# OpenSim2Real/gym-os2r

Hardware: AMD Instinct MI355X
Metric: env-steps/sec (aggregate) monopod balance task (higher is better)
Workload: dtype f64; 1 GPU; C4: 65536 envs/GPU free_hip balancing, ground contact, per-env domain randomisation (C5 = 8 x C4); envs_per_gpu=65536, total_envs=65536, task_mode=free_hip, substeps=10, pgs_exact=12, preroll_steps=1000, contact=True, domain_randomisation=True, actions=U(-1,1) Philox on device, n_ranks_seen=1, splits=1, rollout_steps_per_launch=1

## Files before the change

### gym-os2r_amd/csrc/os2r_device.hpp

```cpp
#pragma once
#include <type_traits>
#include <hip/hip_runtime.h>
#include <stdint.h>

#include "../../include/os2r.h"
#include "os2r_models_gen.hpp"

namespace os2r {

constexpr int kWave = 64;
template <typename T> struct StdSolver { static constexpr int kNormalIters = 2; static constexpr bool kExact = true; };
template <> struct StdSolver<float> { static constexpr int kNormalIters = 2; static constexpr bool kExact = false; };
__host__ __device__ constexpr int warm_first(int) { return 3; }
__host__ __device__ constexpr int sweep_cap_base(int nq) { return nq >= 5 ? 6 : 4; }
constexpr int kExactRounds = 8;
constexpr unsigned kCarryJoints = 0x80000000u;
template <typename T, int NQ_> struct SolverCarry {
  unsigned act = 0u;
  T ln[NQ_] = {}, lx[NQ_] = {}, ly[NQ_] = {}, lf[NQ_] = {};
};
template <typename T> __host__ __device__ constexpr int std_iters(int nq) { return sizeof(T) == 8 ? sweep_cap_base(nq) + kExactRounds : 20; }
template <typename T> __host__ __device__ inline bool is_std_solver(int iters, int normal_iters, int exact, int nq) {
  return iters == std_iters<T>(nq) && normal_iters == StdSolver<T>::kNormalIters && (exact > 0) == StdSolver<T>::kExact;
}
// ... 240 lines not shown
template <typename T> __device__ __forceinline__ T comp(V3<T> a, int k) { return k == 0 ? a.x : (k == 1 ? a.y : a.z); }
template <typename T> __device__ __forceinline__ void add_comp(V3<T>& a, int k, T v) {
  if (k == 0) a.x += v; else if (k == 1) a.y += v; else a.z += v;
}
template <typename T> __device__ __forceinline__ V3<T> rmul(const T (&R)[9], V3<T> v) {
  return {R[0] * v.x + R[1] * v.y + R[2] * v.z, R[3] * v.x + R[4] * v.y + R[5] * v.z, R[6] * v.x + R[7] * v.y + R[8] * v.z};
}
template <typename T> __device__ __forceinline__ V3<T> rtmul(const T (&R)[9], V3<T> v) {
  return {R[0] * v.x + R[3] * v.y + R[6] * v.z, R[1] * v.x + R[4] * v.y + R[7] * v.z, R[2] * v.x + R[5] * v.y + R[8] * v.z};
}

__device__ __forceinline__ double sqrt_t(double x) { return sqrt(x); }
__device__ __forceinline__ float sqrt_t(float x) { return sqrtf(x); }
__device__ __forceinline__ bool sincos_in_range(double x) { return fabs(x) < 8.2e5; }
__device__ __forceinline__ bool sincos_in_range(float x) { return fabsf(x) < 200.0f; }
__device__ __forceinline__ void sincos_lib(double x, double& s, double& c) { sincos(x, &s, &c); }
__device__ __forceinline__ void sincos_lib(float x, float& s, float& c) { sincosf(x, &s, &c); }
__device__ __forceinline__ void sincos_fast(float x, float& s, float& c) {
  const float k = __builtin_rintf(x * 0.636619772f);
  float r = __builtin_fmaf(-k, 1.5703125f, x);
  r = __builtin_fmaf(-k, 4.837512969970703125e-4f, r);
  r = __builtin_fmaf(-k, 7.54978995489188e-8f, r);
  const float z = r * r;
  float ps = -1.9515295891e-4f;
  ps = __builtin_fmaf(ps, z, 8.3321608736e-3f);
  ps = __builtin_fmaf(ps, z, -1.6666654611e-1f);
  const float sr = __builtin_fmaf(r * z, ps, r);
  float pc = 2.443315711809948e-5f;
  pc = __builtin_fmaf(pc, z, -1.388731625493765e-3f);
  pc = __builtin_fmaf(pc, z, 4.166664568298827e-2f);
  const float cr = __builtin_fmaf(z * z, pc, __builtin_fmaf(-0.5f, z, 1.0f));
  const int n = (int)k;
  const float a = (n & 1) ? cr : sr, b = (n & 1) ? sr : cr;
  s = (n & 2) ? -a : a;
  c = ((n + 1) & 2) ? -b : b;
}
__device__ __forceinline__ void sincos_fast(double x, double& s, double& c) {
  const double k = __builtin_rint(x * 0x1.45f306dc9c883p-1);
  double r = __builtin_fma(-k, 0x1.921fb54442d18p+0, x);
  r = __builtin_fma(-k, 0x1.1a62633145c07p-54, r);
  const double z = r * r;
  double ps = 0x1.5d93a5acfd57cp-33;
  ps = __builtin_fma(ps, z, -0x1.ae5e68a2b9cebp-26);
  ps = __builtin_fma(ps, z, 0x1.71de357b1fe7dp-19);
  ps = __builtin_fma(ps, z, -0x1.a01a019c161d5p-13);
  ps = __builtin_fma(ps, z, 0x1.111111110f8a6p-7);
  ps = __builtin_fma(ps, z, -0x1.5555555555549p-3);
  const double sr = __builtin_fma(r * z, ps, r);
  double pc = -0x1.8fae9be8838d4p-37;
  pc = __builtin_fma(pc, z, 0x1.1ee9ebdb4b1c4p-29);
  pc = __builtin_fma(pc, z, -0x1.27e4f809c52adp-22);
  pc = __builtin_fma(pc, z, 0x1.a01a019cb1590p-16);
  pc = __builtin_fma(pc, z, -0x1.6c16c16c15177p-10);
  pc = __builtin_fma(pc, z, 0x1.555555555554cp-5);
  const double cr = __builtin_fma(z * z, pc, __builtin_fma(-0.5, z, 1.0));
  const int n = (int)k;
  const double a = (n & 1) ? cr : sr, b = (n & 1) ? sr : cr;
  s = (n & 2) ? -a : a;
  c = ((n + 1) & 2) ? -b : b;
}

__device__ __forceinline__ double rcp_t(double x) {
  double r = __builtin_amdgcn_rcp(x);
  r = __builtin_fma(__builtin_fma(-x, r, 1.0), r, r);
  r = __builtin_fma(__builtin_fma(-x, r, 1.0), r, r);
  return r;
}
__device__ __forceinline__ float rcp_t(float x) {
  float r = __builtin_amdgcn_rcpf(x);
  return __builtin_fmaf(__builtin_fmaf(-x, r, 1.0f), r, r);
}
__device__ __forceinline__ double rsqrt_t(double x) {
  double r = __builtin_amdgcn_rsq(x);
  r = r * __builtin_fma(-0.5 * x * r, r, 1.5);
  r = r * __builtin_fma(-0.5 * x * r, r, 1.5);
  return r;
}
__device__ __forceinline__ float rsqrt_t(float x) {
  float r = __builtin_amdgcn_rsqf(x);
  return r * __builtin_fmaf(-0.5f * x * r, r, 1.5f);
}

__device__ __forceinline__ double fmax_t(double a, double b) { return fmax(a, b); }
__device__ __forceinline__ float fmax_t(float a, float b) { return fmaxf(a, b); }
__device__ __forceinline__ double fmin_t(double a, double b) { return fmin(a, b); }
__device__ __forceinline__ float fmin_t(float a, float b) { return fminf(a, b); }
__device__ __forceinline__ double fma_t(double a, double b, double c) { return __builtin_fma(a, b, c); }
__device__ __forceinline__ float fma_t(float a, float b, float c) { return __builtin_fmaf(a, b, c); }
__device__ __forceinline__ double fabs_t(double x) { return fabs(x); }
__device__ __forceinline__ float fabs_t(float x) { return fabsf(x); }

__device__ __forceinline__ bool finite_t(double x) {
  asm volatile("" : "+v"(x));
  return ((__double_as_longlong(x) >> 52) & 0x7ff) != 0x7ff;
}
__device__ __forceinline__ bool finite_t(float x) {
  asm volatile("" : "+v"(x));
  return ((__float_as_int(x) >> 23) & 0xff) != 0xff;
}

template <typename T> __device__ __forceinline__ V3<T> symmul(const T (&S)[6], V3<T> v) {
  return {S[0] * v.x + S[1] * v.y + S[2] * v.z, S[1] * v.x + S[3] * v.y + S[4] * v.z, S[2] * v.x + S[4] * v.y + S[5] * v.z};
}

template <typename T>
struct ArtInertia {
  T A[6];
  T H[9];
  T M[6];
};

template <typename T> __device__ __forceinline__ void rot_general(const T (&R)[9], const T (&B)[9], T (&out)[9]) {
  T t[9];
#pragma unroll
  for (int i = 0; i < 3; ++i)
#pragma unroll
    for (int j = 0; j < 3; ++j) t[3 * i + j] = R[3 * i] * B[j] + R[3 * i + 1] * B[3 + j] + R[3 * i + 2] * B[6 + j];
#pragma unroll
  for (int i = 0; i < 3; ++i)
#pragma unroll
    for (int j = 0; j < 3; ++j) out[3 * i + j] = t[3 * i] * R[3 * j] + t[3 * i + 1] * R[3 * j + 1] + t[3 * i + 2] * R[3 * j + 2];
}
template <typename T> __device__ __forceinline__ void rot_sym(const T (&R)[9], const T (&S)[6], T (&out)[6]) {
  const T B[9] = {S[0], S[1], S[2], S[1], S[3], S[4], S[2], S[4], S[5]};
  T t[9];
#pragma unroll
  for (int i = 0; i < 3; ++i)
#pragma unroll
    for (int j = 0; j < 3; ++j) t[3 * i + j] = R[3 * i] * B[j] + R[3 * i + 1] * B[3 + j] + R[3 * i + 2] * B[6 + j];
  int k = 0;
#pragma unroll
  for (int i = 0; i < 3; ++i)
#pragma unroll
    for (int j = i; j < 3; ++j) out[k++] = t[3 * i] * R[3 * j] + t[3 * i + 1] * R[3 * j + 1] + t[3 * i + 2] * R[3 * j + 2];
}

template <typename T, typename MD, bool DR>
struct Params;
template <typename T, typename MD>
struct Params<T, MD, false> {
  MD m;
  T g;
  __device__ __forceinline__ T mass(int i) const { return m.mass(i); }
  __device__ __forceinline__ T damping(int i) const { return m.damping(i); }
  __device__ __forceinline__ T friction(int i) const { return m.friction(i); }
  __device__ __forceinline__ T mu(int i) const { return m.mu(i); }
  __device__ __forceinline__ T gravity() const { return g; }
};
template <typename T, typename MD>
struct Params<T, MD, true> {
  MD m;
  const T* slots;
  T g;
  static constexpr int NQ = MD::NQ;
  __device__ __forceinline__ T mass(int i) const { return slots[(0 * NQ + i) * kWave]; }
  __device__ __forceinline__ T damping(int i) const { return slots[(1 * NQ + i) * kWave]; }
  __device__ __forceinline__ T friction(int i) const { return slots[(2 * NQ + i) * kWave]; }
  __device__ __forceinline__ T mu(int i) const { return slots[(3 * NQ + i) * kWave]; }
  __device__ __forceinline__ T gravity() const { return g; }
};

constexpr int kStamps = 32;
#if defined(OS2R_STAMPS) && defined(OS2R_STAMPS_LIGHT)
#define OS2R_STAMP(idx) do { } while (0)
#elif defined(OS2R_STAMPS)
#define OS2R_STAMP(idx)                                                                        \
  do {                                                                                         \
    __builtin_amdgcn_sched_barrier(0);                                                         \
    unsigned long long t_;                                                                     \
    asm volatile("s_memtime %0\n\ts_waitcnt lgkmcnt(0)" : "=s"(t_)::"memory");                 \
    __builtin_amdgcn_sched_barrier(0);                                                         \
    stamps[idx] += t_ - stamp_prev;                                                            \
    stamp_prev = t_;                                                                           \
  } while (0)
#elif defined(OS2R_PHASE_MARKS)
#define OS2R_STAMP(idx) asm volatile("s_nop 15\n\ts_nop %0\n\ts_nop %1" :: "i"((idx) % 8), "i"((idx) / 8) : "memory")
#else
#define OS2R_STAMP(idx) do { } while (0)
#endif

#ifdef OS2R_ISA_MARKS
#define OS2R_ISA_MARK(n) asm volatile("s_nop " #n ::: "memory")
#else
#define OS2R_ISA_MARK(n) do { } while (0)
#endif

constexpr int kPinVmem = 0x1 | 0x2 | 0x4 | 0x8 | 0x80 | 0x100 | 0x200 | 0x400;

constexpr int kPinDs = 0x1 | 0x2 | 0x4 | 0x8 | 0x10 | 0x20 | 0x40 | 0x400;

__device__ __forceinline__ double opaque(double x) { asm volatile("" : "+v"(x)); return x; }
__device__ __forceinline__ float opaque(float x) { asm volatile("" : "+v"(x)); return x; }

template <typename T> __device__ __forceinline__ T pick3(int k, T a, T b, T c) { return k == 0 ? a : (k == 1 ? b : c); }

template <typename T, typename MD>
__device__ __forceinline__ void joint_rotation(const MD& md, int i, T s_, T c_, T (&R)[9]) {
  const T s = opaque(s_), c = opaque(c_);
  const int ax = md.axis(i);
  const int ca = ax == 0 ? 1 : (ax == 1 ? 2 : 0);
  const int cb = ax == 0 ? 2 : (ax == 1 ? 0 : 1);
#pragma unroll
  for (int r = 0; r < 3; ++r) {
    const T fa = md.rfix(i, 3 * r + ca), fb = md.rfix(i, 3 * r + cb);
    const T keep = md.rfix(i, 3 * r + ax), va = c * fa + s * fb, vb = c * fb - s * fa;
#pragma unroll
    for (int j = 0; j < 3; ++j) R[3 * r + j] = j == ax ? keep : (j == ca ? va : vb);
  }
}

template <unsigned CMASK, int NB>
__device__ __forceinline__ constexpr int next_cand_body(int b) {
  for (int k = b + 1; k < NB; ++k)
    if ((CMASK >> k) & 1u) return k;
  return NB;
}
template <int B, int NB, unsigned CMASK, typename F>
__device__ __forceinline__ bool for_body(int b, F&& f) {
  if constexpr (B < NB) {
    if constexpr (((CMASK >> B) & 1u) && __builtin_popcount(CMASK >> B) <= 3) {
      if (b == B) { f(std::integral_constant<int, B>{}); return true; }
    }
    return for_body<B + 1, NB, CMASK>(b, f);
  } else {
    return false;
  }
}

enum { kSolverBoth = 0, kSolverExact = 1, kSolverSweeps = 2 };
template <typename T, typename MD, bool CONTACT, bool DR, bool COUNT = false, int SOLVER = kSolverBoth>
__device__ __forceinline__ void substep(const MD& md, const Params<T, MD, DR>& par,
                                        T (&q)[MD::NQ], T (&qd)[MD::NQ], T (&sn)[MD::NQ], T (&cs)[MD::NQ], bool first_iteration,
                                        T tau_hip, T tau_knee, T dt, T erp,
                                        T max_erv, T margin, int pgs_iters, int pgs_normal_iters, int pgs_exact, T pgs_tol, T* __restrict__ lds,
                                        const T* __restrict__ cand_lds, ModelPtr<T> mconst, WorkCounts& wc, SolverCarry<T, MD::NQ>& carry
#ifdef OS2R_STAMPS
                                        , unsigned long long (&stamps)[kStamps], unsigned long long& stamp_prev
#endif
                                        ) {
  constexpr int NQ = MD::NQ;
  constexpr unsigned CMASK = CONTACT ? MD::CMASK : 0u;
  const T inv_dt = rcp_t(dt);
  const T m_first = par.mass(NQ - 1), damp_first = par.damping(NQ - 1);
  __builtin_amdgcn_sched_barrier(DR ? kPinDs : kPinVmem);
  {
    bool ok = true, small = !first_iteration;
#pragma unroll
    for (int i = 0; i < NQ; ++i) { ok = ok && sincos_in_range(q[i]); small = small && fabs_t(dt * qd[i]) < T(0.06); }
    if constexpr (COUNT) wc.full_sincos += __ballot(!small) != 0ull ? 1u : 0u;
    if (small) {
#pragma unroll
      for (int i = 0; i < NQ; ++i) {
        const T d = dt * qd[i], z = d * d;
        T p = fma_t(z, T(-1.0 / 39916800.0), T(1.0 / 362880.0));
        p = fma_t(z, p, T(-1.0 / 5040.0));
        p = fma_t(z, p, T(1.0 / 120.0));
        p = fma_t(z, p, T(-1.0 / 6.0));
        const T sd = fma_t(d * z, p, d);
        T r = fma_t(z, T(-1.0 / 3628800.0), T(1.0 / 40320.0));
        r = fma_t(z, r, T(-1.0 / 720.0));
        r = fma_t(z, r, T(1.0 / 24.0));
        r = fma_t(z, r, T(-0.5));
        const T cm = z * r;
        const T s0 = sn[i], c0 = cs[i];
        sn[i] = s0 + fma_t(c0, sd, s0 * cm);
        cs[i] = c0 + fma_t(-s0, sd, c0 * cm);
      }
    } else if (ok) {
#pragma unroll
      for (int i = 0; i < NQ; ++i) sincos_fast(q[i], sn[i], cs[i]);
    } else {
#pragma unroll
      for (int i = 0; i < NQ; ++i) sincos_lib(q[i], sn[i], cs[i]);
    }
  }

  OS2R_STAMP(0);
  const int lane_ = threadIdx.x;
  auto L = [&](int slot) -> T& { return lds[slot * kWave + lane_]; };
  constexpr int kUa = 0, kUl = 3 * NQ, kDi = 6 * NQ, kU = 7 * NQ;
  auto ldv = [&](int base, int i) { return mk(L(base + 3 * i), L(base + 3 * i + 1), L(base + 3 * i + 2)); };
  auto stv = [&](int base, int i, V3<T> x) { L(base + 3 * i) = x.x; L(base + 3 * i + 1) = x.y; L(base + 3 * i + 2) = x.z; };

  V3<T> wv[NQ], vv[NQ];
  {
    V3<T> w = mk<T>(0, 0, 0), v = mk<T>(0, 0, 0);
#pragma unroll
    for (int i = 0; i < NQ; ++i) {
      if (i > 0) {
        const V3<T> r = mk(md.rpos(i, 0), md.rpos(i, 1), md.rpos(i, 2));
        T Ri[9];
        joint_rotation<T>(md, i, sn[i], cs[i], Ri);
        const V3<T> wn = rtmul(Ri, w);
        v = rtmul(Ri, v + cross(w, r));
        w = wn;
      }
      add_comp(w, md.axis(i), qd[i]);
      wv[i] = w;
      vv[i] = v;
    }
  }

  OS2R_STAMP(12);
  {
    ArtInertia<T> acc;
    V3<T> pn, pf;
    T m_next = m_first, damp_next = damp_first;
#pragma unroll
    for (int i = NQ - 1; i >= 0; --i) {
      const int ax = md.axis(i);
      const V3<T> w = wv[i], v = vv[i];
      const T m = m_next;
      const T damp = damp_next;
      if (i > 0) {
        m_next = par.mass(i - 1);
        damp_next = par.damping(i - 1);
        __builtin_amdgcn_sched_barrier(DR ? kPinDs : kPinVmem);
      }
      const V3<T> cm = mk(md.com(i, 0), md.com(i, 1), md.com(i, 2));
      const V3<T> h = m * cm;
      ArtInertia<T> I;
      I.A[0] = md.icom(i, 0) + m * (cm.y * cm.y + cm.z * cm.z);
      I.A[1] = md.icom(i, 1) - m * cm.x * cm.y;
      I.A[2] = md.icom(i, 2) - m * cm.x * cm.z;
      I.A[3] = md.icom(i, 3) + m * (cm.x * cm.x + cm.z * cm.z);
      I.A[4] = md.icom(i, 4) - m * cm.y * cm.z;
      I.A[5] = md.icom(i, 5) + m * (cm.x * cm.x + cm.y * cm.y);
      I.H[0] = 0; I.H[1] = -h.z; I.H[2] = h.y;
      I.H[3] = h.z; I.H[4] = 0; I.H[5] = -h.x;
      I.H[6] = -h.y; I.H[7] = h.x; I.H[8] = 0;
      I.M[0] = m; I.M[1] = 0; I.M[2] = 0; I.M[3] = m; I.M[4] = 0; I.M[5] = m;
      const V3<T> nI = symmul(I.A, w) + cross(h, v);
      const V3<T> fI = m * v - cross(h, w);
      V3<T> pAn = cross(w, nI) + cross(v, fI);
      V3<T> pAf = cross(w, fI);
      if (i < NQ - 1) {
#pragma unroll
        for (int k = 0; k < 6; ++k) { I.A[k] += acc.A[k]; I.M[k] += acc.M[k]; }
#pragma unroll
        for (int k = 0; k < 9; ++k) I.H[k] += acc.H[k];
        pAn = pAn + pn;
        pAf = pAf + pf;
      }
      const V3<T> Ua = mk(pick3(ax, I.A[0], I.A[1], I.A[2]), pick3(ax, I.A[1], I.A[3], I.A[4]), pick3(ax, I.A[2], I.A[4], I.A[5]));
      const V3<T> Ul = mk(pick3(ax, I.H[0], I.H[3], I.H[6]), pick3(ax, I.H[1], I.H[4], I.H[7]), pick3(ax, I.H[2], I.H[5], I.H[8]));
      const T D = comp(Ua, ax) + dt * damp;
      const T Dinv = rcp_t(D);
      T tau = T(0);
      if (i == md.act_dof(0)) tau = tau_hip;
      if (i == md.act_dof(1)) tau = tau_knee;
      const T u = tau - damp * qd[i] - comp(pAn, ax);
      stv(kUa, i, Ua);
      stv(kUl, i, Ul);
      L(kDi + i) = Dinv;
      L(kU + i) = u;
      if (i > 0) {
        const V3<T> ka = Dinv * Ua, kl = Dinv * Ul;
        ArtInertia<T> Ia;
        Ia.A[0] = I.A[0] - ka.x * Ua.x; Ia.A[1] = I.A[1] - ka.x * Ua.y; Ia.A[2] = I.A[2] - ka.x * Ua.z;
        Ia.A[3] = I.A[3] - ka.y * Ua.y; Ia.A[4] = I.A[4] - ka.y * Ua.z; Ia.A[5] = I.A[5] - ka.z * Ua.z;
        Ia.H[0] = I.H[0] - ka.x * Ul.x; Ia.H[1] = I.H[1] - ka.x * Ul.y; Ia.H[2] = I.H[2] - ka.x * Ul.z;
        Ia.H[3] = I.H[3] - ka.y * Ul.x; Ia.H[4] = I.H[4] - ka.y * Ul.y; Ia.H[5] = I.H[5] - ka.y * Ul.z;
        Ia.H[6] = I.H[6] - ka.z * Ul.x; Ia.H[7] = I.H[7] - ka.z * Ul.y; Ia.H[8] = I.H[8] - ka.z * Ul.z;
        Ia.M[0] = I.M[0] - kl.x * Ul.x; Ia.M[1] = I.M[1] - kl.x * Ul.y; Ia.M[2] = I.M[2] - kl.x * Ul.z;
        Ia.M[3] = I.M[3] - kl.y * Ul.y; Ia.M[4] = I.M[4] - kl.y * Ul.z; Ia.M[5] = I.M[5] - kl.z * Ul.z;
        V3<T> sq = mk<T>(0, 0, 0);
        add_comp(sq, ax, qd[i]);
        const V3<T> ca = cross(w, sq), cl = cross(v, sq);
        const V3<T> Hc = mk(Ia.H[0] * cl.x + Ia.H[1] * cl.y + Ia.H[2] * cl.z, Ia.H[3] * cl.x + Ia.H[4] * cl.y + Ia.H[5] * cl.z,
                            Ia.H[6] * cl.x + Ia.H[7] * cl.y + Ia.H[8] * cl.z);
        const V3<T> Htc = mk(Ia.H[0] * ca.x + Ia.H[3] * ca.y + Ia.H[6] * ca.z, Ia.H[1] * ca.x + Ia.H[4] * ca.y + Ia.H[7] * ca.z,
                             Ia.H[2] * ca.x + Ia.H[5] * ca.y + Ia.H[8] * ca.z);
        const T ud = u * Dinv;
        const V3<T> pan = pAn + symmul(Ia.A, ca) + Hc + ud * Ua;
        const V3<T> paf = pAf + Htc + symmul(Ia.M, cl) + ud * Ul;
        const V3<T> r = mk(md.rpos(i, 0), md.rpos(i, 1), md.rpos(i, 2));
        T Ri[9];
        joint_rotation<T>(md, i, sn[i], cs[i], Ri);
        T Ar[6], Hr[9], Mr[6];
        rot_sym(Ri, Ia.A, Ar);
        rot_general(Ri, Ia.H, Hr);
        rot_sym(Ri, Ia.M, Mr);
        const T Mf[9] = {Mr[0], Mr[1], Mr[2], Mr[1], Mr[3], Mr[4], Mr[2], Mr[4], Mr[5]};
        T Hs[9];
#pragma unroll
        for (int j = 0; j < 3; ++j) {
          const V3<T> col = cross(r, mk(Mf[j], Mf[3 + j], Mf[6 + j]));
          Hs[j] = Hr[j] + col.x; Hs[3 + j] = Hr[3 + j] + col.y; Hs[6 + j] = Hr[6 + j] + col.z;
        }
        V3<T> x0[3], x1[3];
#pragma unroll
        for (int k = 0; k < 3; ++k) {
          x0[k] = cross(r, mk(Hr[3 * k], Hr[3 * k + 1], Hr[3 * k + 2]));
          x1[k] = cross(r, mk(Hs[3 * k], Hs[3 * k + 1], Hs[3 * k + 2]));
        }
        acc.A[0] = Ar[0] + x0[0].x + x1[0].x;
        acc.A[1] = Ar[1] + x0[1].x + x1[0].y;
        acc.A[2] = Ar[2] + x0[2].x + x1[0].z;
        acc.A[3] = Ar[3] + x0[1].y + x1[1].y;
        acc.A[4] = Ar[4] + x0[2].y + x1[1].z;
        acc.A[5] = Ar[5] + x0[2].z + x1[2].z;
#pragma unroll
        for (int k = 0; k < 9; ++k) acc.H[k] = Hs[k];
#pragma unroll
        for (int k = 0; k < 6; ++k) acc.M[k] = Mr[k];
        pf = rmul(Ri, paf);
        pn = rmul(Ri, pan) + cross(r, pf);
      }
      OS2R_STAMP(13 + (NQ - 1 - i));
    }
  }

  T vs[NQ];
  T hu[2], hd[2];
  V3<T> hua[2], hul[2];
  {
    V3<T> aa = mk<T>(0, 0, 0), al = mk<T>(0, 0, -par.gravity());
    auto request = [&](int i, int b) { hu[b] = L(kU + i); hua[b] = ldv(kUa, i); hul[b] = ldv(kUl, i); hd[b] = L(kDi + i); };
    auto arrived = [&](int b) {
      asm volatile("" : "+v"(hu[b]), "+v"(hd[b]), "+v"(hua[b].x), "+v"(hua[b].y), "+v"(hua[b].z), "+v"(hul[b].x), "+v"(hul[b].y), "+v"(hul[b].z));
      asm volatile("" ::: "memory");
    };
    request(0, 0);
#pragma unroll
    for (int i = 0; i < NQ; ++i) {
      const int b = i & 1;
      arrived(b);
      if (i + 1 < NQ) request(i + 1, b ^ 1);
      const int ax = md.axis(i);
      const V3<T> r = mk(md.rpos(i, 0), md.rpos(i, 1), md.rpos(i, 2));
      V3<T> sq = mk<T>(0, 0, 0);
      add_comp(sq, ax, qd[i]);
      T Ri[9];
      joint_rotation<T>(md, i, sn[i], cs[i], Ri);
      const V3<T> pa_ = rtmul(Ri, aa);
      const V3<T> pl_ = rtmul(Ri, al + cross(aa, r));
      aa = pa_ + cross(wv[i], sq);
      al = pl_ + cross(vv[i], sq);
      const T qdd = (hu[b] - dot(hua[b], aa) - dot(hul[b], al)) * hd[b];
      add_comp(aa, ax, qdd);
      vs[i] = qd[i] + dt * qdd;
    }
  }

  OS2R_STAMP(1);
  constexpr int NB = NQ;
  constexpr int kLc = 0;
  auto Lcs = [&](int i, int k) -> T& { return L(kLc + i * (i + 1) / 2 + k); };
  T Lc[NQ][NQ];
  T Ldi[NQ];
  {
    T uk[NQ][NQ];
    V3<T> pn_[NQ], pf_[NQ];
    V3<T> mUa[2], mUl[2];
    T mdi[2];
    auto request_m = [&](int i, int b) { mUa[b] = ldv(kUa, i); mUl[b] = ldv(kUl, i); mdi[b] = L(kDi + i); };
    auto arrived_m = [&](int b) {
      asm volatile("" : "+v"(mdi[b]), "+v"(mUa[b].x), "+v"(mUa[b].y), "+v"(mUa[b].z), "+v"(mUl[b].x), "+v"(mUl[b].y), "+v"(mUl[b].z));
      asm volatile("" ::: "memory");
    };
    constexpr bool kAhead = sizeof(T) == 8;
    if constexpr (kAhead) { mUa[(NQ - 1) & 1] = hua[(NQ - 1) & 1]; mUl[(NQ - 1) & 1] = hul[(NQ - 1) & 1]; mdi[(NQ - 1) & 1] = hd[(NQ - 1) & 1]; }
#pragma unroll
    for (int i = NQ - 1; i >= 0; --i) {
      if constexpr (kAhead) {
        if (i < NQ - 1) arrived_m(i & 1);
        if (i > 0) { request_m(i - 1, (i - 1) & 1); __builtin_amdgcn_sched_barrier(kPinDs); }
      } else {
        request_m(i, i & 1);
      }
      const V3<T> Ua = mUa[i & 1], Ul = mUl[i & 1];
      const T di = mdi[i & 1];
      uk[i][i] = T(1);
      if (i < NQ - 1) {
        const V3<T> r = mk(md.rpos(i + 1, 0), md.rpos(i + 1, 1), md.rpos(i + 1, 2));
        T Ri[9];
        joint_rotation<T>(md, i + 1, sn[i + 1], cs[i + 1], Ri);
#pragma unroll
        for (int k = i + 1; k < NQ; ++k) {
          const V3<T> f = rmul(Ri, pf_[k]);
          const V3<T> n = rmul(Ri, pn_[k]) + cross(r, f);
          uk[k][i] = -comp(n, md.axis(i));
          if (i > 0) {
            const T s_ = uk[k][i] * di;
            pn_[k] = n + s_ * Ua;
            pf_[k] = f + s_ * Ul;
          }
        }
      }
      if (i > 0) {
        pn_[i] = di * Ua;
        pf_[i] = di * Ul;
      }
      Ldi[i] = rsqrt_t(di);
      const T sdi = di * Ldi[i];
#pragma unroll
      for (int r = i; r < NQ; ++r) Lc[r][i] = r == i ? sdi : uk[r][i] * sdi;
    }
  }
  OS2R_STAMP(19);

  OS2R_STAMP(2);
  T fb[NQ];
  T mub[NB];
#pragma unroll
  for (int j = 0; j < NQ; ++j) fb[j] = par.friction(j);
#pragma unroll
  for (int b = 0; b < NB; ++b) mub[b] = ((CMASK >> b) & 1u) ? par.mu(b) : T(0);
  __builtin_amdgcn_sched_barrier(DR ? kPinDs : kPinVmem);
  T y[NQ];
  T idj[NQ];
#pragma unroll
  for (int j = 0; j < NQ; ++j) {
    T mjj = 0;
#pragma unroll
    for (int k = 0; k <= j; ++k) { mjj += Lc[j][k] * Lc[j][k]; Lcs(j, k) = Lc[j][k]; }
    idj[j] = mjj > T(0) ? rcp_t(mjj) : T(0);
  }
#pragma unroll
  for (int i = 0; i < NQ; ++i) {
    T acc_ = vs[i];
#pragma unroll
    for (int k = 0; k < i; ++k) acc_ -= Lc[i][k] * y[k];
    y[i] = opaque(acc_ * Ldi[i]);
  }
  constexpr bool kStdExact = sizeof(T) == 8 && SOLVER == kSolverExact && MD::kStatic;
  constexpr bool kParkY0 = sizeof(T) == 8 && !kStdExact && (SOLVER != kSolverSweeps || !MD::kStatic);
  constexpr int kY0Slot = NQ * (NQ + 1) / 2 + 3 * NQ + NQ;
  static_assert(kY0Slot + NQ <= 8 * NQ, "per-lane LDS slots");
  T y0[NQ];
#pragma unroll
  for (int i = 0; i < NQ; ++i) {
    if constexpr (kParkY0) L(kY0Slot + i) = y[i];
    else y0[i] = y[i];
  }

  OS2R_STAMP(3);
  T dn[NB], dx[NB], dy[NB], erv[NB];
  T Gr[NB][3][NQ];
  bool act[NB];
  bool wave_act[NB];
#pragma unroll
  for (int b = 0; b < NB; ++b) { act[b] = false; wave_act[b] = false; }
  if (CMASK != 0u) {
    T Rw[9], ow[3];
    V3<T> aw[NQ], jo[NQ];
#pragma unroll
    for (int b = 0; b < NB; ++b) {
      constexpr int CHS = 4;
      T bA[3 * CHS], bB[3 * CHS];
      auto request = [&](int kk, int kend, T (&d)[3 * CHS]) {
#pragma unroll
        for (int j = 0; j < 3 * CHS; ++j) d[j] = (kk + j / 3 < kend) ? mconst->cand_p[kk + j / 3][j % 3] : T(0);
      };
      if constexpr (MD::kStatic) {
        if ((CMASK >> b) & 1u) {
          request(md.cand_begin(b), md.cand_begin(b + 1), bA);
          asm volatile("" ::: "memory");
        }
      }
      const V3<T> r = mk(md.rpos(b, 0), md.rpos(b, 1), md.rpos(b, 2));
      T Rb[9];
      joint_rotation<T>(md, b, sn[b], cs[b], Rb);
      if (b == 0) {
#pragma unroll
        for (int k = 0; k < 9; ++k) Rw[k] = Rb[k];
        ow[0] = r.x; ow[1] = r.y; ow[2] = r.z;
      } else {
        const V3<T> t = rmul(Rw, r);
        ow[0] += t.x; ow[1] += t.y; ow[2] += t.z;
        T n[9];
#pragma unroll
        for (int i = 0; i < 3; ++i)
#pragma unroll
          for (int j = 0; j < 3; ++j) n[3 * i + j] = Rw[3 * i] * Rb[j] + Rw[3 * i + 1] * Rb[3 + j] + Rw[3 * i + 2] * Rb[6 + j];
#pragma unroll
        for (int k = 0; k < 9; ++k) Rw[k] = n[k];
      }
      const int ax = md.axis(b);
      aw[b] = mk(pick3(ax, Rw[0], Rw[1], Rw[2]), pick3(ax, Rw[3], Rw[4], Rw[5]), pick3(ax, Rw[6], Rw[7], Rw[8]));
      jo[b] = mk(ow[0], ow[1], ow[2]);
      if (!((CMASK >> b) & 1u)) continue;
      OS2R_STAMP(4);
      const int k0 = md.cand_begin(b), k1 = md.cand_begin(b + 1);
      T W = 0, sx = 0, sy = 0, sz = 0;
      const T zc = Rw[6] * md.cand_center(b, 0) + Rw[7] * md.cand_center(b, 1) + Rw[8] * md.cand_center(b, 2) + ow[2];
      const bool near = zc - md.cand_radius(b) < margin;
      if constexpr (MD::kStatic) {
#pragma unroll
        for (int j = 0; j < 3 * CHS; ++j) asm volatile("" : "+s"(bA[j]));
        asm volatile("" ::: "memory");
      }
      if constexpr (COUNT) wc.scanned += __ballot(near) != 0ull ? 1u : 0u;
      if (__ballot(near) != 0ull)
      {
        constexpr int CH = 4;
        auto fetch = [&](int k, T (&d)[3 * CH]) {
#pragma unroll
          for (int j = 0; j < 3 * CH; ++j) d[j] = cand_lds[3 * k + j];
        };
        auto consume = [&](const T (&d)[3 * CH]) {
#pragma unroll
          for (int c = 0; c < CH; ++c) {
            const T px = d[3 * c], py = d[3 * c + 1], pz = d[3 * c + 2];
            const T z = Rw[6] * px + Rw[7] * py + Rw[8] * pz + ow[2];
            const T wgt = fmax_t(margin - z, T(0));
            W += wgt; sx += wgt * px; sy += wgt * py; sz += wgt * pz;
          }
        };
        if constexpr (MD::kStatic) {
          const T mo = margin - ow[2];
          auto arrived = [&](T (&d)[3 * CH]) {
#pragma unroll
            for (int j = 0; j < 3 * CH; ++j) asm volatile("" : "+s"(d[j]));
            asm volatile("" ::: "memory");
          };
          const int ga = MD::cand_group_axis(b), a1 = (ga + 1) % 3, a2 = (ga + 2) % 3;
          T S[3] = {T(0), T(0), T(0)};
          T Wg = T(0), pg = T(0), base = mo;
          auto weigh = [&](const T (&d)[3 * CH], int kk) {
#pragma unroll
            for (int c = 0; c < CH; ++c) {
              if (kk + c < k1) {
                if (MD::cand_starts_run(b, kk + c, ga)) {
                  W += Wg; S[ga] = fma_t(pg, Wg, S[ga]);
                  Wg = T(0); pg = d[3 * c + ga];
                  base = fma_t(-Rw[6 + ga], pg, mo);
                }
                const T p1 = d[3 * c + a1], p2 = d[3 * c + a2];
                const T mz = fma_t(-Rw[6 + a1], p1, fma_t(-Rw[6 + a2], p2, base));
                const T wgt = fmax_t(mz, T(0));
                Wg += wgt; S[a1] = fma_t(wgt, p1, S[a1]); S[a2] = fma_t(wgt, p2, S[a2]);
              }
            }
          };
          static_assert(CH == CHS, "chunk size of the request issued ahead");
#pragma unroll
          for (int kk = k0; kk < k1; kk += 2 * CH) {
            arrived(bA);
            if (kk + CH < k1) request(kk + CH, k1, bB);
            weigh(bA, kk);
            if (kk + CH < k1) {
              arrived(bB);
              if (kk + 2 * CH < k1) request(kk + 2 * CH, k1, bA);
              weigh(bB, kk + CH);
            }
          }
          W += Wg; S[ga] = fma_t(pg, Wg, S[ga]);
          sx = S[0]; sy = S[1]; sz = S[2];
        } else {
        T bufA[3 * CH], bufB[3 * CH];
        int k = k0;
        const int kpair = k0 + ((k1 - k0) / (2 * CH)) * (2 * CH);
        if (k < kpair) {
          fetch(k, bufA);
#pragma unroll 1
          for (; k < kpair; k += 2 * CH) {
            fetch(k + CH, bufB);
            consume(bufA);
            if (k + 2 * CH < kpair) fetch(k + 2 * CH, bufA);
            consume(bufB);
          }
        }
#pragma unroll 1
        for (; k < k1; ++k) {
          const T px = cand_lds[3 * k], py = cand_lds[3 * k + 1], pz = cand_lds[3 * k + 2];
          const T z = Rw[6] * px + Rw[7] * py + Rw[8] * pz + ow[2];
          const T wgt = fmax_t(margin - z, T(0));
          W += wgt; sx += wgt * px; sy += wgt * py; sz += wgt * pz;
        }
        }
      }
      OS2R_STAMP(5);
      act[b] = W > T(0);
      wave_act[b] = __ballot(act[b]) != 0ull;
      if constexpr (COUNT) { wc.row_bodies += wave_act[b] ? 1u : 0u; wc.lane_contacts += (unsigned)__popcll(__ballot(act[b])); }
      if (wave_act[b]) {
        T lcb[NQ][NQ];
#pragma unroll
        for (int j = 0; j < NQ; ++j)
#pragma unroll
          for (int k = 0; k < NQ; ++k)
            if (j <= b && k <= j) lcb[j][k] = Lcs(j, k);
        __builtin_amdgcn_sched_barrier(kPinDs);
        const T iw = act[b] ? rcp_t(W) : T(0);
        const V3<T> pc = mk(sx * iw, sy * iw, sz * iw);
        const V3<T> pw = rmul(Rw, pc) + jo[b];
        const T gap = pw.z;
        const T e = erp * (-gap) * inv_dt;
        erv[b] = gap >= T(0) ? -gap * inv_dt : (e > max_erv ? max_erv : e);
        T Jn[NQ], Jx[NQ], Jy[NQ];
#pragma unroll
        for (int j = 0; j < NQ; ++j) {
          if (j <= b) {
            const V3<T> c = cross(aw[j], pw - jo[j]);
            Jx[j] = c.x; Jy[j] = c.y; Jn[j] = c.z;
          }
        }
        T sdn = 0, sdx = 0, sdy = 0;
#pragma unroll
        for (int k = 0; k < NQ; ++k) {
          if (k <= b) {
            T gn = 0, gx = 0, gy = 0;
#pragma unroll
            for (int j = k; j < NQ; ++j)
              if (j <= b) { const T l = lcb[j][k]; gn += Jn[j] * l; gx += Jx[j] * l; gy += Jy[j] * l; }
            Gr[b][0][k] = gn; Gr[b][1][k] = gx; Gr[b][2][k] = gy;
            sdn += gn * gn; sdx += gx * gx; sdy += gy * gy;
          }
        }
        dn[b] = (act[b] && sdn > T(0)) ? rcp_t(sdn) : T(0);
        dx[b] = (act[b] && sdx > T(0)) ? rcp_t(sdx) : T(0);
        dy[b] = (act[b] && sdy > T(0)) ? rcp_t(sdy) : T(0);
      }
    }
  }

  OS2R_STAMP(6);
  T ln[NB], lx[NB], ly[NB], lf[NQ];
#pragma unroll
  for (int b = 0; b < NB; ++b) { ln[b] = 0; lx[b] = 0; ly[b] = 0; }
#pragma unroll
  for (int j = 0; j < NQ; ++j) lf[j] = 0;
#pragma unroll
  for (int j = 0; j < NQ; ++j) {
    fb[j] = opaque(fb[j] * dt);
    idj[j] = fb[j] > T(0) ? idj[j] : T(0);
  }

  T moved = T(0);
  auto contact_row = [&](int b, int row, T target, T rd, T& l, T lo, T hi, bool upper, bool measure) {
    T g[NQ];
    T res = -target;
#pragma unroll
    for (int k = 0; k < NQ; ++k)
      if (k <= b) { g[k] = Gr[b][row][k]; res = fma_t(g[k], y[k], res); }
    T lam = fma_t(-res, rd, l);
    lam = lam < lo ? lo : lam;
    if (upper) lam = lam > hi ? hi : lam;
    const T dl = lam - l;
    l = lam;
    if (measure) moved = fma_t(fabs_t(res), fabs_t(dl), moved);
#pragma unroll
    for (int k = 0; k < NQ; ++k)
      if (k <= b) y[k] = fma_t(g[k], dl, y[k]);
  };
  auto joint_rows = [&](bool measure) {
#pragma unroll
    for (int j = 0; j < NQ; ++j) {
      T res = Lc[j][0] * y[0];
#pragma unroll
      for (int k = 1; k < NQ; ++k)
        if (k <= j) res = fma_t(Lc[j][k], y[k], res);
      T lam = fma_t(-res, idj[j], lf[j]);
// ... 436 lines not shown
```

Before: 494.7 million env-steps/s.

## Fuse mass-matrix factor computation into the articulated-inertia inward pass

For static f64 models with domain randomisation and four DOFs, the Cholesky-like factor (Lc, Ldi) is now built during the backward articulated-body sweep. Propagated unit-force columns are transformed alongside the inertia accumulation, so the separate second inward pass is skipped, along with its reloads of Ua/Ul/Dinv from the scratch store. The cost is higher register pressure from carrying the cuk, cpn and cpf arrays through the sweep, which could hurt occupancy.

```diff
diff --git a/gym-os2r_amd/csrc/os2r_device.hpp b/gym-os2r_amd/csrc/os2r_device.hpp
--- a/gym-os2r_amd/csrc/os2r_device.hpp
+++ b/gym-os2r_amd/csrc/os2r_device.hpp
@@ -566,6 +566,11 @@
   }
 
   OS2R_STAMP(12);
+  constexpr bool kFusedInward = sizeof(T) == 8 && MD::kStatic && DR && NQ == 4;
+  T Lc[NQ][NQ];
+  T Ldi[NQ];
+  T cuk[NQ][NQ];
+  V3<T> cpn[NQ], cpf[NQ];
   {
     ArtInertia<T> acc;
     V3<T> pn, pf;
@@ -618,6 +623,27 @@
       stv(kUl, i, Ul);
       L(kDi + i) = Dinv;
       L(kU + i) = u;
+      if constexpr (kFusedInward) {
+        cuk[i][i] = T(1);
+#pragma unroll
+        for (int k = i + 1; k < NQ; ++k) {
+          const V3<T> n = cpn[k], f = cpf[k];
+          cuk[k][i] = -comp(n, ax);
+          if (i > 0) {
+            const T s_ = cuk[k][i] * Dinv;
+            cpn[k] = n + s_ * Ua;
+            cpf[k] = f + s_ * Ul;
+          }
+        }
+        if (i > 0) {
+          cpn[i] = Dinv * Ua;
+          cpf[i] = Dinv * Ul;
+        }
+        Ldi[i] = rsqrt_t(Dinv);
+        const T sdi = Dinv * Ldi[i];
+#pragma unroll
+        for (int r = i; r < NQ; ++r) Lc[r][i] = r == i ? sdi : cuk[r][i] * sdi;
+      }
       if (i > 0) {
         const V3<T> ka = Dinv * Ua, kl = Dinv * Ul;
         ArtInertia<T> Ia;
@@ -670,6 +696,14 @@
         for (int k = 0; k < 6; ++k) acc.M[k] = Mr[k];
         pf = rmul(Ri, paf);
         pn = rmul(Ri, pan) + cross(r, pf);
+        if constexpr (kFusedInward) {
+#pragma unroll
+          for (int k = i; k < NQ; ++k) {
+            const V3<T> f = rmul(Ri, cpf[k]);
+            cpn[k] = rmul(Ri, cpn[k]) + cross(r, f);
+            cpf[k] = f;
+          }
+        }
       }
       OS2R_STAMP(13 + (NQ - 1 - i));
     }
@@ -711,9 +745,7 @@
   constexpr int NB = NQ;
   constexpr int kLc = 0;
   auto Lcs = [&](int i, int k) -> T& { return L(kLc + i * (i + 1) / 2 + k); };
-  T Lc[NQ][NQ];
-  T Ldi[NQ];
-  {
+  if constexpr (!kFusedInward) {
     T uk[NQ][NQ];
     V3<T> pn_[NQ], pf_[NQ];
     V3<T> mUa[2], mUl[2];
```

Result: no change. 495.2 million env-steps/s (median of 4 runs) (+0.1%).
